# Rita-zi/WavTokenizer

Hardware: AMD Instinct MI355X
Metric: audio-seconds/sec encode+decode, 24 kHz 3 s clips (higher is better)
Workload: dtype f32 (split-f16 x3 products)

## Files before the change

### wavtokenizer_amd/csrc/lstm_persist.hip

```cpp
#include "common.h"

#include <stdlib.h>

namespace wt {

typedef float f32x4p __attribute__((ext_vector_type(4)));
typedef _Float16 f16x8p __attribute__((ext_vector_type(8)));

static constexpr int PW = 12;
static constexpr int HROW = 2 * 2048;
static constexpr int HPITCH = HROW;
template <bool SMALL> __device__ __forceinline__ int lp_swz(int row) { return (SMALL ? 2 * row : row) & 15; }
static constexpr long SPIN_LIMIT_DF = 1L << 20;
template <bool SMALL> struct LpCfg { static constexpr int NLDS = SMALL ? 8 : 6, HROWS = SMALL ? 8 : 16, POLL = SMALL ? 3 : 1; };

__device__ __forceinline__ float sigm_p(float x) { return __builtin_amdgcn_rcpf(1.f + __expf(-x)); }
__device__ __forceinline__ float tanh_p(float x) {
    const float ax = fabsf(x);
    const float e = __expf(-2.f * ax);
    const float t = ax < 0.04f ? ax * (1.f - ax * ax * (1.f / 3.f)) : (1.f - e) * __builtin_amdgcn_rcpf(1.f + e);
    return copysignf(t, x);
}

__device__ __forceinline__ unsigned has_mark(unsigned d) { return (~d - 0x00010001u) & d & 0x80008000u; }
__device__ __forceinline__ _Float16 no_mark(_Float16 v) {
    const unsigned short b = __builtin_bit_cast(unsigned short, v);
    return __builtin_bit_cast(_Float16, (unsigned short)(b == 0xFFFFu ? 0x7E00u : b));
}

#define LP_TRACE(ph) do { if (TRACE && tr_on && s >= 64 && s < 72) { \
    const unsigned long long tt = __builtin_amdgcn_s_memrealtime(); \
    if (lane == 0) { a.ctl[520 + ((s - 64) * 6 + (ph)) * 2] = (unsigned)tt; a.ctl[521 + ((s - 64) * 6 + (ph)) * 2] = (unsigned)(tt >> 32); } } } while (0)
template <bool SMALL, bool TRACE = false>
__global__ __launch_bounds__(64 * PW) void lstm_persist_kernel(const LstmPersistArgs a) {
    constexpr int NBUF = 3;
    constexpr int NLDS = LpCfg<SMALL>::NLDS, HROWS = LpCfg<SMALL>::HROWS;
    extern __shared__ __attribute__((aligned(16))) char sm_p[];
    char* hst = sm_p;
    float* gbuf = reinterpret_cast<float*>(sm_p + HROWS * HPITCH);
    f32x4p* wlds = reinterpret_cast<f32x4p*>(sm_p + HROWS * HPITCH + 3 * 4 * 16 * 17 * sizeof(float)) + (threadIdx.x >> 6) * NLDS * 64 + (threadIdx.x & 63);
    __shared__ unsigned s_xcc, s_w, s_stop;
    const int tid = threadIdx.x, lane = tid & 63, wave = tid >> 6;
    const int role = wave >> 2, ntile = wave & 3;
    const int li = lane & 15, lk = lane >> 4;
    if (tid == 0) {
        const unsigned xcc = __builtin_amdgcn_s_getreg(20 | (3 << 11)) & 7;
        s_xcc = xcc;
        s_w = __hip_atomic_fetch_add(a.ctl + xcc * 32, 1u, __ATOMIC_RELAXED, __HIP_MEMORY_SCOPE_WORKGROUP) + 1u;
        s_stop = 0;
    }
    __syncthreads();
    const int xcc = (int)s_xcc, w = (int)s_w;
    if (w >= 32) return;
    const int H = 512, B = a.B, L = a.L;
    const int c0g = xcc * a.Bx;
    const int nb = B - c0g < a.Bx ? B - c0g : a.Bx;
    if (nb <= 0) return;
    unsigned* err = a.ctl + 512;
    char* hx = reinterpret_cast<char*>(a.hx) + (size_t)xcc * (NBUF * 2 * 16 * 2048);
    const __amdgpu_buffer_rsrc_t rsH = __builtin_amdgcn_make_buffer_rsrc(hx, 0, NBUF * 2 * 16 * 2048, 0x00020000);

    f16x8p wh[16], wl[16 - NLDS];
    {
        const f32x4p* wp = reinterpret_cast<const f32x4p*>(a.Wp) + ((((size_t)role * 32 + w) * 4 + ntile) * 16 * 2) * 64 + lane;
#pragma unroll
        for (int blk = 0; blk < 16; ++blk) {
            wh[blk] = __builtin_bit_cast(f16x8p, wp[(blk * 2 + 0) * 64]);
            if (blk < 16 - NLDS) wl[blk] = __builtin_bit_cast(f16x8p, wp[(blk * 2 + 1) * 64]);
            else wlds[(blk - (16 - NLDS)) * 64] = wp[(blk * 2 + 1) * 64];
        }
    }
    const int c_layer = tid >> 8, c_clip = (tid >> 4) & 15, c_unit = tid & 15;
    const bool c_thr = tid < 512 && c_clip < nb;
    const int c_nt = c_unit >> 2, c_u4 = c_unit & 3;
    const int j = 16 * w + c_unit;
    const long gclip = c0g + c_clip;
    float cst = 0.f;

    for (int e = tid; e < HROWS * HPITCH / 16; e += 64 * PW) reinterpret_cast<f32x4p*>(hst)[e] = (f32x4p){0.f, 0.f, 0.f, 0.f};
    __syncthreads();
    const long spin_limit_df = SPIN_LIMIT_DF >> a.dbg_spin_shift;
    const bool tr_on = TRACE && xcc == 0 && w == 0 && __builtin_amdgcn_readfirstlane(wave) == 0;
    for (int s = 0; s <= L; ++s) {
        LP_TRACE(0);
        float xg[4] = {0.f, 0.f, 0.f, 0.f};
        float xs = 0.f;
        if (c_thr && c_layer == 0 && s < L) {
#pragma unroll
            for (int g = 0; g < 4; ++g) xg[g] = a.xg0[((long)s * B + gclip) * (4 * H) + 64 * w + 16 * c_nt + g * 4 + c_u4];
        }
        if (c_thr && c_layer == 1 && s >= 1) {
            xs = a.x[(gclip * L + (s - 1)) * H + j];
#pragma unroll
            for (int g = 0; g < 4; ++g) xg[g] = a.b1[64 * w + 16 * c_nt + g * 4 + c_u4];
        }

        {
            const int rb = (s + 2) % 3, tot = 2 * nb * 128;
            constexpr int POLL = LpCfg<SMALL>::POLL;
            for (int e0 = tid; e0 < tot; e0 += POLL * 64 * PW) {
                f32x4p v[POLL];
                unsigned need = 0;
#pragma unroll
                for (int it = 0; it < POLL; ++it) {
                    const int e = e0 + it * 64 * PW;
                    if (e < tot && s >= 1 + (e >> 7) / nb) need |= 1u << it;
                }
                unsigned pend = need;
                long spin = 0;
                while (pend) {
#pragma unroll
                    for (int it = 0; it < POLL; ++it)
                        if (pend >> it & 1) {
                            const int e = e0 + it * 64 * PW;
                            const int c16 = e & 127, lc = e >> 7, layer = lc / nb, clip = lc - layer * nb;
                            v[it] = __builtin_bit_cast(f32x4p, __builtin_amdgcn_raw_buffer_load_b128(
                                        rsH, ((rb * 2 + layer) * 16 + clip) * 2048 + c16 * 16, 0, 16 ));
                        }
                    unsigned still = 0;
#pragma unroll
                    for (int it = 0; it < POLL; ++it)
                        if (pend >> it & 1) {
                            const unsigned m = has_mark(__builtin_bit_cast(unsigned, v[it].x)) | has_mark(__builtin_bit_cast(unsigned, v[it].y)) |
                                               has_mark(__builtin_bit_cast(unsigned, v[it].z)) | has_mark(__builtin_bit_cast(unsigned, v[it].w));
                            if (m) still |= 1u << it;
                        }
                    pend = still;
                    if (pend) {
                        if (++spin > spin_limit_df || ((spin & 1023) == 0 && __hip_atomic_load(err, __ATOMIC_RELAXED, __HIP_MEMORY_SCOPE_AGENT) == 1u)) {
                            __hip_atomic_store(err, 1u, __ATOMIC_RELAXED, __HIP_MEMORY_SCOPE_AGENT);
                            if (a.status) __hip_atomic_fetch_or(a.status, (unsigned)WT_STATUS_LSTM, __ATOMIC_RELAXED, __HIP_MEMORY_SCOPE_AGENT);
                            s_stop = 1;
                            break;
                        }
                        __builtin_amdgcn_s_sleep(1);
                    }
                }
#pragma unroll
                for (int it = 0; it < POLL; ++it) {
                    const int e = e0 + it * 64 * PW;
                    if (e < tot) {
                        const int c16 = e & 127, lc = e >> 7, layer = lc / nb, clip = lc - layer * nb;
                        *reinterpret_cast<f32x4p*>(hst + clip * HPITCH + layer * 2048 + ((c16 ^ lp_swz<SMALL>(clip)) * 16)) =
                            (need >> it & 1) ? v[it] : (f32x4p){0.f, 0.f, 0.f, 0.f};
                    }
                }
            }
            LP_TRACE(1);
            __syncthreads();
            LP_TRACE(2);
            if (s_stop) return;
            if (c_thr) {
                unsigned short* mrow = reinterpret_cast<unsigned short*>(hx + ((((s + 1) % 3) * 2 + c_layer) * 16 + c_clip) * 2048);
                mrow[(j >> 5) * 64 + (j & 31)] = 0xFFFFu;
                mrow[(j >> 5) * 64 + 32 + (j & 31)] = 0xFFFFu;
            }
        }
        {
            const bool act = role == 0 ? (s < L) : (s >= 1);
            if (act && SMALL) {
                const int ach = (lk + ((li & 8) ? 4 : 0)) ^ lp_swz<SMALL>(li & 7);
                const char* ap0 = hst + (li & 7) * HPITCH + (role == 2 ? 2048 : 0) + (ach & 7) * 16;
                const char* ape = ap0 + (ach >> 3) * 128;
                const char* apo = ap0 + (1 ^ (ach >> 3)) * 128;
                const bool arow = (li & 7) < nb;
                f32x4p accm = {0.f, 0.f, 0.f, 0.f}, accc = accm;
                f16x8p a1b[2] = {{0, 0, 0, 0, 0, 0, 0, 0}, {0, 0, 0, 0, 0, 0, 0, 0}};
                if (arow) a1b[0] = *reinterpret_cast<const f16x8p*>(ape);
#pragma unroll
                for (int blk = 0; blk < 16; ++blk) {
                    if (blk + 1 < 16 && arow) a1b[(blk + 1) & 1] = *reinterpret_cast<const f16x8p*>((((blk + 1) & 1) ? apo : ape) + ((blk + 1) >> 1) * 256);
                    const f16x8p a1 = a1b[blk & 1];
                    const f16x8p wlb = blk < 16 - NLDS ? wl[blk < 16 - NLDS ? blk : 0]
                                                       : __builtin_bit_cast(f16x8p, wlds[(blk - (16 - NLDS)) * 64]);
                    accm = __builtin_amdgcn_mfma_f32_16x16x32_f16(a1, wh[blk], accm, 0, 0, 0);
                    accc = __builtin_amdgcn_mfma_f32_16x16x32_f16(a1, wlb, accc, 0, 0, 0);
                }
                float* gb = gbuf + ((role * 4 + ntile) * 16) * 17;
#pragma unroll
                for (int r = 0; r < 4; ++r) {
                    const float c2 = __shfl_down(accm[r], 32, 64);
                    if (lk < 2) gb[(4 * lk + r) * 17 + li] = accm[r] + (accc[r] + c2) * (1.f / 2048.f);
                }
            } else if (act) {
                const int ch_h = lk ^ lp_swz<SMALL>(li);
                const char* ap0 = hst + li * HPITCH + (role == 2 ? 2048 : 0) + (ch_h & 7) * 16;
                const char* ape = ap0 + (ch_h >> 3) * 128;
                const char* apo = ap0 + (1 ^ (ch_h >> 3)) * 128;
                const int lo_d = (ch_h & 4) ? -64 : 64;
                f32x4p accm = {0.f, 0.f, 0.f, 0.f}, acc_hl = accm, acc_lh = accm;
                {
                    f16x8p ahb[2];
                    ahb[0] = *reinterpret_cast<const f16x8p*>(ape);
#pragma unroll
                    for (int blk = 0; blk < 16; ++blk) {
                        if (blk + 1 < 16) ahb[(blk + 1) & 1] = *reinterpret_cast<const f16x8p*>((((blk + 1) & 1) ? apo : ape) + ((blk + 1) >> 1) * 256);
                        const f16x8p ah = ahb[blk & 1];
                        const f16x8p wlb = blk < 16 - NLDS ? wl[blk < 16 - NLDS ? blk : 0]
                                                           : __builtin_bit_cast(f16x8p, wlds[(blk - (16 - NLDS)) * 64]);
                        accm = __builtin_amdgcn_mfma_f32_16x16x32_f16(ah, wh[blk], accm, 0, 0, 0);
                        acc_hl = __builtin_amdgcn_mfma_f32_16x16x32_f16(ah, wlb, acc_hl, 0, 0, 0);
                    }
                }
                {
                    f16x8p alb[2];
                    alb[0] = *reinterpret_cast<const f16x8p*>(ape + lo_d);
#pragma unroll
                    for (int blk = 0; blk < 16; ++blk) {
                        if (blk + 1 < 16) alb[(blk + 1) & 1] = *reinterpret_cast<const f16x8p*>((((blk + 1) & 1) ? apo : ape) + ((blk + 1) >> 1) * 256 + lo_d);
                        acc_lh = __builtin_amdgcn_mfma_f32_16x16x32_f16(alb[blk & 1], wh[blk], acc_lh, 0, 0, 0);
                    }
                }
                float* gb = gbuf + ((role * 4 + ntile) * 16) * 17;
#pragma unroll
                for (int r = 0; r < 4; ++r) gb[(4 * lk + r) * 17 + li] = accm[r] + (acc_hl[r] + acc_lh[r]) * (1.f / 2048.f);
            }
        }
        LP_TRACE(3);
        __syncthreads();
        LP_TRACE(4);
        if (c_thr && (c_layer == 0 ? (s < L) : (s >= 1))) {
            float pre[4];
#pragma unroll
            for (int g = 0; g < 4; ++g) {
                const int col = g * 4 + c_u4;
                if (c_layer == 0) pre[g] = gbuf[((0 * 4 + c_nt) * 16 + c_clip) * 17 + col] + xg[g];
                else pre[g] = (gbuf[((1 * 4 + c_nt) * 16 + c_clip) * 17 + col] + gbuf[((2 * 4 + c_nt) * 16 + c_clip) * 17 + col]) + xg[g];
            }
            const float ig = sigm_p(pre[0]), fg = sigm_p(pre[1]), gg = tanh_p(pre[2]), og = sigm_p(pre[3]);
            cst = fg * cst + ig * gg;
            const float h = og * tanh_p(cst);
            _Float16* hrow = reinterpret_cast<_Float16*>(hx + (((s % 3) * 2 + c_layer) * 16 + c_clip) * 2048);
            const _Float16 hh = (_Float16)h;
            const _Float16 hl = (_Float16)((h - (float)hh) * 2048.f);
            __builtin_amdgcn_s_waitcnt(0);
            hrow[(j >> 5) * 64 + (j & 31)] = no_mark(hh);
            hrow[(j >> 5) * 64 + 32 + (j & 31)] = no_mark(hl);
            if (c_layer == 1) {
                const int t = s - 1;
                const float yv = h + xs;
                const float o = a.elu_out ? (yv > 0.f ? yv : __expf(yv) - 1.f) : yv;
                float* yrow = a.y + (gclip * L + t) * H;
                if (a.out_s32) {
                    if (fabsf(o) >= 65504.f && a.status)
                        __hip_atomic_fetch_or(a.status, (unsigned)WT_STATUS_RANGE, __ATOMIC_RELAXED, __HIP_MEMORY_SCOPE_AGENT);
                    _Float16* yp = reinterpret_cast<_Float16*>(yrow) + ((j >> 5) * 64 + (j & 31));
                    const _Float16 oh = (_Float16)o;
                    yp[0] = oh;
                    yp[32] = (_Float16)((o - (float)oh) * 2048.f);
                } else {
                    yrow[j] = o;
                }
            }
        }
        LP_TRACE(5);
    }
}

size_t lstm_persist_hx_bytes() { return (size_t)8 * 3 * 2 * 16 * 2048; }
size_t lstm_persist_ctl_bytes() { return 1024 * sizeof(unsigned); }

int launch_lstm_persist(const LstmPersistArgs& a, hipStream_t stream) {
    if (a.H != 512) { set_error("lstm_persist: built for hidden size 512"); return -1; }
    if (a.B < 1 || a.Bx < 1 || a.Bx > 16 || 8 * a.Bx < a.B) { set_error("lstm_persist: at most 16 clips per XCD (B <= 128)"); return -1; }
    static PerDeviceOnce attr_once;
    constexpr size_t smem_big = (size_t)16 * HPITCH + (size_t)3 * 4 * 16 * 17 * sizeof(float) + (size_t)PW * LpCfg<false>::NLDS * 1024;
    constexpr size_t smem_small = (size_t)8 * HPITCH + (size_t)3 * 4 * 16 * 17 * sizeof(float) + (size_t)PW * LpCfg<true>::NLDS * 1024;
    static_assert(smem_big + 64 <= 160 * 1024 && smem_small + 64 <= 160 * 1024, "LDS budget");
    if (int rc = attr_once.run([&]() -> int {
        WT_HIP_CHECK(hipFuncSetAttribute(reinterpret_cast<const void*>(lstm_persist_kernel<false>), hipFuncAttributeMaxDynamicSharedMemorySize, (int)smem_big));
        WT_HIP_CHECK(hipFuncSetAttribute(reinterpret_cast<const void*>(lstm_persist_kernel<true>), hipFuncAttributeMaxDynamicSharedMemorySize, (int)smem_small));
#ifdef WT_LAB
        WT_HIP_CHECK(hipFuncSetAttribute(reinterpret_cast<const void*>(lstm_persist_kernel<false, true>), hipFuncAttributeMaxDynamicSharedMemorySize, (int)smem_big));
        WT_HIP_CHECK(hipFuncSetAttribute(reinterpret_cast<const void*>(lstm_persist_kernel<true, true>), hipFuncAttributeMaxDynamicSharedMemorySize, (int)smem_small));
#endif
        return 0;
    })) return rc;
    const bool small = a.Bx <= 8;
    LstmPersistArgs b = a;
    if (!b.status) b.status = g_launch.status;
    const char* fault = lab_env("WT_LSTM_PERSIST_FAULT");
    const bool forced = fault && fault[0] == '1';
    if (forced) b.dbg_spin_shift = 8;
    const dim3 grid(forced ? 248 : 256), block(64 * PW);
#ifdef WT_LAB
    if (a.data_flag & 4) {
        if (small) hipLaunchKernelGGL((lstm_persist_kernel<true, true>), grid, block, smem_small, stream, b);
        else hipLaunchKernelGGL((lstm_persist_kernel<false, true>), grid, block, smem_big, stream, b);
    } else
#endif
    {
        if (small) hipLaunchKernelGGL((lstm_persist_kernel<true>), grid, block, smem_small, stream, b);
        else hipLaunchKernelGGL((lstm_persist_kernel<false>), grid, block, smem_big, stream, b);
    }
    WT_HIP_CHECK(hipGetLastError());
    if (LstmForm* f = g_launch.lstm_form) {
        f->kernel = 0; f->small = small ? 1 : 0; f->Bx = a.Bx; f->grid[0] = grid.x; f->grid[1] = grid.y; f->block = block.x;
        f->lds = (unsigned)(small ? smem_small : smem_big);
        ++f->launches;
    }
    return 0;
}

}
```

Baseline: 38340.

## Software-pipeline LDS reads with explicit waitcnt in persistent LSTM step

Rewrites the per-step MFMA loop of the persistent LSTM kernel to issue LDS operand reads through inline ds_read_b128 with fixed offsets. Each read is placed three blocks ahead and guarded by a computed lgkmcnt wait, and the large and small paths are unified into one 32- or 16-block sequence. The polling loop now always issues all POLL loads, decodes the layer with a compare instead of a division and uses a wider POLL for the big config. Cell indices and output offsets are precomputed before the barriers to cut register pressure, and the small config keeps one fewer weight fragment in LDS. Hand-written waitcnt counts are fragile and could break if the compiler reorders LDS operations, and lab-only ablation variants are added.

```diff
diff --git a/wavtokenizer_amd/csrc/lstm_persist.hip b/wavtokenizer_amd/csrc/lstm_persist.hip
--- a/wavtokenizer_amd/csrc/lstm_persist.hip
+++ b/wavtokenizer_amd/csrc/lstm_persist.hip
@@ -1,6 +1,8 @@
 #include "common.h"
 
 #include <stdlib.h>
+
+#include <utility>
 
 namespace wt {
 
@@ -12,7 +14,34 @@
 static constexpr int HPITCH = HROW;
 template <bool SMALL> __device__ __forceinline__ int lp_swz(int row) { return (SMALL ? 2 * row : row) & 15; }
 static constexpr long SPIN_LIMIT_DF = 1L << 20;
-template <bool SMALL> struct LpCfg { static constexpr int NLDS = SMALL ? 8 : 6, HROWS = SMALL ? 8 : 16, POLL = SMALL ? 3 : 1; };
+template <bool SMALL> struct LpCfg { static constexpr int NLDS = SMALL ? 7 : 6, HROWS = SMALL ? 8 : 16, POLL = 3; };
+
+__device__ __forceinline__ unsigned lds_addr(const void* p) { return (unsigned)(size_t)p; }
+template <int OFF> __device__ __forceinline__ void lds_read16(f16x8p& d, unsigned addr) {
+    static_assert(OFF >= 0 && OFF < 65536, "ds offset field");
+    asm volatile("ds_read_b128 %0, %1 offset:%2" : "=v"(d) : "v"(addr), "n"(OFF));
+}
+template <int N> __device__ __forceinline__ void lds_wait(f16x8p& x) { asm volatile("s_waitcnt lgkmcnt(%1)" : "+v"(x) : "n"(N)); }
+template <int N> __device__ __forceinline__ void lds_wait(f16x8p& x, f16x8p& y) { asm volatile("s_waitcnt lgkmcnt(%2)" : "+v"(x), "+v"(y) : "n"(N)); }
+constexpr int lp_ord_a(int k) { return k < 3 ? k : 3 + 2 * (k - 3); }
+constexpr int lp_ord_w(int k) { return 3 + 2 * (k - 2) + 1; }
+constexpr int lp_younger(int v, int NV, int W0) {
+    int last = lp_ord_a(v);
+    if (v >= W0 && v < 16 && lp_ord_w(v) > last) last = lp_ord_w(v);
+    int n = 0;
+    for (int k = 0; k < NV; ++k) if ((k < 3 || k - 3 < v) && lp_ord_a(k) > last) ++n;
+    for (int k = W0; k < 16; ++k) if (k - 2 < v && lp_ord_w(k) > last) ++n;
+    return n;
+}
+__device__ __forceinline__ int lp_fresh(int t) { asm volatile("" : "+v"(t)); return t; }
+#define LP_CELL_IDS \
+    const int c_t = lp_fresh(tid), c_layer = c_t >> 8, c_clip = (c_t >> 4) & 15, c_unit = c_t & 15; \
+    const bool c_thr = c_t < 512 && c_clip < nb; \
+    const int c_nt = c_unit >> 2, c_u4 = c_unit & 3; \
+    const int j = 16 * w + c_unit;                        \
+    const long gclip = c0g + c_clip; \
+    (void)c_layer; (void)c_nt; (void)c_u4; (void)j; (void)gclip
+template <class F, int... I> __device__ __forceinline__ void lp_blocks(F&& f, std::integer_sequence<int, I...>) { (f(std::integral_constant<int, I>{}), ...); }
 
 __device__ __forceinline__ float sigm_p(float x) { return __builtin_amdgcn_rcpf(1.f + __expf(-x)); }
 __device__ __forceinline__ float tanh_p(float x) {
@@ -30,19 +59,17 @@
 
 #define LP_TRACE(ph) do { if (TRACE && tr_on && s >= 64 && s < 72) { \
     const unsigned long long tt = __builtin_amdgcn_s_memrealtime(); \
-    if (lane == 0) { a.ctl[520 + ((s - 64) * 6 + (ph)) * 2] = (unsigned)tt; a.ctl[521 + ((s - 64) * 6 + (ph)) * 2] = (unsigned)(tt >> 32); } } } while (0)
-template <bool SMALL, bool TRACE = false>
+    if ((tid & 63) == 0) { a.ctl[520 + ((s - 64) * 6 + (ph)) * 2] = (unsigned)tt; a.ctl[521 + ((s - 64) * 6 + (ph)) * 2] = (unsigned)(tt >> 32); } } } while (0)
+template <bool SMALL, bool TRACE = false, int ABL = 0>
 __global__ __launch_bounds__(64 * PW) void lstm_persist_kernel(const LstmPersistArgs a) {
     constexpr int NBUF = 3;
     constexpr int NLDS = LpCfg<SMALL>::NLDS, HROWS = LpCfg<SMALL>::HROWS;
     extern __shared__ __attribute__((aligned(16))) char sm_p[];
     char* hst = sm_p;
     float* gbuf = reinterpret_cast<float*>(sm_p + HROWS * HPITCH);
-    f32x4p* wlds = reinterpret_cast<f32x4p*>(sm_p + HROWS * HPITCH + 3 * 4 * 16 * 17 * sizeof(float)) + (threadIdx.x >> 6) * NLDS * 64 + (threadIdx.x & 63);
+    char* wlds0 = sm_p + HROWS * HPITCH + 3 * 4 * 16 * 17 * sizeof(float);
     __shared__ unsigned s_xcc, s_w, s_stop;
     const int tid = threadIdx.x, lane = tid & 63, wave = tid >> 6;
-    const int role = wave >> 2, ntile = wave & 3;
-    const int li = lane & 15, lk = lane >> 4;
     if (tid == 0) {
         const unsigned xcc = __builtin_amdgcn_s_getreg(20 | (3 << 11)) & 7;
         s_xcc = xcc;
@@ -62,7 +89,9 @@
 
     f16x8p wh[16], wl[16 - NLDS];
     {
+        const int role = wave >> 2, ntile = wave & 3;
         const f32x4p* wp = reinterpret_cast<const f32x4p*>(a.Wp) + ((((size_t)role * 32 + w) * 4 + ntile) * 16 * 2) * 64 + lane;
+        f32x4p* wlds = reinterpret_cast<f32x4p*>(wlds0) + wave * NLDS * 64 + lane;
 #pragma unroll
         for (int blk = 0; blk < 16; ++blk) {
             wh[blk] = __builtin_bit_cast(f16x8p, wp[(blk * 2 + 0) * 64]);
@@ -70,186 +99,204 @@
             else wlds[(blk - (16 - NLDS)) * 64] = wp[(blk * 2 + 1) * 64];
         }
     }
-    const int c_layer = tid >> 8, c_clip = (tid >> 4) & 15, c_unit = tid & 15;
-    const bool c_thr = tid < 512 && c_clip < nb;
-    const int c_nt = c_unit >> 2, c_u4 = c_unit & 3;
-    const int j = 16 * w + c_unit;
-    const long gclip = c0g + c_clip;
     float cst = 0.f;
 
     for (int e = tid; e < HROWS * HPITCH / 16; e += 64 * PW) reinterpret_cast<f32x4p*>(hst)[e] = (f32x4p){0.f, 0.f, 0.f, 0.f};
     __syncthreads();
-    const long spin_limit_df = SPIN_LIMIT_DF >> a.dbg_spin_shift;
+    const int spin_limit_df = (int)(SPIN_LIMIT_DF >> a.dbg_spin_shift);
     const bool tr_on = TRACE && xcc == 0 && w == 0 && __builtin_amdgcn_readfirstlane(wave) == 0;
     for (int s = 0; s <= L; ++s) {
         LP_TRACE(0);
         float xg[4] = {0.f, 0.f, 0.f, 0.f};
         float xs = 0.f;
-        if (c_thr && c_layer == 0 && s < L) {
-#pragma unroll
-            for (int g = 0; g < 4; ++g) xg[g] = a.xg0[((long)s * B + gclip) * (4 * H) + 64 * w + 16 * c_nt + g * 4 + c_u4];
-        }
-        if (c_thr && c_layer == 1 && s >= 1) {
-            xs = a.x[(gclip * L + (s - 1)) * H + j];
-#pragma unroll
-            for (int g = 0; g < 4; ++g) xg[g] = a.b1[64 * w + 16 * c_nt + g * 4 + c_u4];
-        }
-
+        unsigned ape, apo, apw;
+        int lo_d;
         {
             const int rb = (s + 2) % 3, tot = 2 * nb * 128;
             constexpr int POLL = LpCfg<SMALL>::POLL;
-            for (int e0 = tid; e0 < tot; e0 += POLL * 64 * PW) {
-                f32x4p v[POLL];
+            for (int e0 = lp_fresh(tid); e0 < tot; e0 += POLL * 64 * PW) {
                 unsigned need = 0;
+                int off[POLL];
 #pragma unroll
                 for (int it = 0; it < POLL; ++it) {
-                    const int e = e0 + it * 64 * PW;
-                    if (e < tot && s >= 1 + (e >> 7) / nb) need |= 1u << it;
-                }
-                unsigned pend = need;
-                long spin = 0;
-                while (pend) {
+                    const int e = e0 + it * 64 * PW, ec = e < tot ? e : tot - 1;
+                    const int c16 = ec & 127, lc = ec >> 7, layer = lc >= nb ? 1 : 0, clip = lc - layer * nb;
+                    off[it] = ((rb * 2 + layer) * 16 + clip) * 2048 + c16 * 16;
+                    if (e < tot && s >= 1 + layer) need |= 1u << it;
+                }
+                f32x4p va[POLL];
+                int spin = 0;
+                while (need) {
 #pragma unroll
                     for (int it = 0; it < POLL; ++it)
-                        if (pend >> it & 1) {
-                            const int e = e0 + it * 64 * PW;
-                            const int c16 = e & 127, lc = e >> 7, layer = lc / nb, clip = lc - layer * nb;
-                            v[it] = __builtin_bit_cast(f32x4p, __builtin_amdgcn_raw_buffer_load_b128(
-                                        rsH, ((rb * 2 + layer) * 16 + clip) * 2048 + c16 * 16, 0, 16 ));
-                        }
+                        va[it] = __builtin_bit_cast(f32x4p, __builtin_amdgcn_raw_buffer_load_b128(rsH, off[it], 0, 16 ));
                     unsigned still = 0;
 #pragma unroll
-                    for (int it = 0; it < POLL; ++it)
-                        if (pend >> it & 1) {
-                            const unsigned m = has_mark(__builtin_bit_cast(unsigned, v[it].x)) | has_mark(__builtin_bit_cast(unsigned, v[it].y)) |
-                                               has_mark(__builtin_bit_cast(unsigned, v[it].z)) | has_mark(__builtin_bit_cast(unsigned, v[it].w));
-                            if (m) still |= 1u << it;
-                        }
-                    pend = still;
-                    if (pend) {
-                        if (++spin > spin_limit_df || ((spin & 1023) == 0 && __hip_atomic_load(err, __ATOMIC_RELAXED, __HIP_MEMORY_SCOPE_AGENT) == 1u)) {
-                            __hip_atomic_store(err, 1u, __ATOMIC_RELAXED, __HIP_MEMORY_SCOPE_AGENT);
-                            if (a.status) __hip_atomic_fetch_or(a.status, (unsigned)WT_STATUS_LSTM, __ATOMIC_RELAXED, __HIP_MEMORY_SCOPE_AGENT);
-                            s_stop = 1;
-                            break;
-                        }
-                        __builtin_amdgcn_s_sleep(1);
-                    }
+                    for (int it = 0; it < POLL; ++it) {
+                        const unsigned m = has_mark(__builtin_bit_cast(unsigned, va[it].x)) | has_mark(__builtin_bit_cast(unsigned, va[it].y)) |
+                                           has_mark(__builtin_bit_cast(unsigned, va[it].z)) | has_mark(__builtin_bit_cast(unsigned, va[it].w));
+                        if (m) still |= 1u << it;
+                    }
+                    if ((ABL & 2) || !(still & need)) break;
+                    if (++spin > spin_limit_df || ((spin & 1023) == 0 && __hip_atomic_load(err, __ATOMIC_RELAXED, __HIP_MEMORY_SCOPE_AGENT) == 1u)) {
+                        __hip_atomic_store(err, 1u, __ATOMIC_RELAXED, __HIP_MEMORY_SCOPE_AGENT);
+                        if (a.status) __hip_atomic_fetch_or(a.status, (unsigned)WT_STATUS_LSTM, __ATOMIC_RELAXED, __HIP_MEMORY_SCOPE_AGENT);
+                        s_stop = 1;
+                        break;
+                    }
+                    __builtin_amdgcn_s_sleep(1);
                 }
 #pragma unroll
                 for (int it = 0; it < POLL; ++it) {
                     const int e = e0 + it * 64 * PW;
                     if (e < tot) {
-                        const int c16 = e & 127, lc = e >> 7, layer = lc / nb, clip = lc - layer * nb;
+                        const int c16 = e & 127, lc = e >> 7, layer = lc >= nb ? 1 : 0, clip = lc - layer * nb;
                         *reinterpret_cast<f32x4p*>(hst + clip * HPITCH + layer * 2048 + ((c16 ^ lp_swz<SMALL>(clip)) * 16)) =
-                            (need >> it & 1) ? v[it] : (f32x4p){0.f, 0.f, 0.f, 0.f};
-                    }
-                }
-            }
+                            (need >> it & 1) ? va[it] : (f32x4p){0.f, 0.f, 0.f, 0.f};
+                    }
+                }
+            }
+            {
+                LP_CELL_IDS;
+                if (c_thr && c_layer == 0 && s < L) {
+#pragma unroll
+                    for (int g = 0; g < 4; ++g) xg[g] = a.xg0[((long)s * B + gclip) * (4 * H) + 64 * w + 16 * c_nt + g * 4 + c_u4];
+                }
+                if (c_thr && c_layer == 1 && s >= 1) {
+                    xs = a.x[(gclip * L + (s - 1)) * H + j];
+#pragma unroll
+                    for (int g = 0; g < 4; ++g) xg[g] = a.b1[64 * w + 16 * c_nt + g * 4 + c_u4];
+                }
+            }
+            int m_off;
+            {
+                LP_CELL_IDS;
+                m_off = c_thr ? ((((s + 1) % 3) * 2 + c_layer) * 16 + c_clip) * 2048 + ((j >> 5) * 64 + (j & 31)) * 2 : -1;
+            }
+            {
+                const int tp = lp_fresh(tid), role = tp >> 8, li = tp & 15, lk = (tp >> 4) & 3;
+                const int row = SMALL ? (li & 7) : li;
+                const int ch = (SMALL ? lk + ((li & 8) ? 4 : 0) : lk) ^ lp_swz<SMALL>(row);
+                const unsigned ap0 = lds_addr(hst + row * HPITCH + (role == 2 ? 2048 : 0) + (ch & 7) * 16);
+                ape = ap0 + (ch >> 3) * 128;
+                apo = ap0 + (1 ^ (ch >> 3)) * 128;
+                lo_d = (ch & 4) ? -64 : 64;
+                apw = lds_addr(wlds0) + (tp >> 6) * (NLDS * 1024) + (tp & 63) * 16;
+            }
+            asm volatile("" : "+v"(m_off), "+v"(ape), "+v"(apo), "+v"(lo_d), "+v"(apw));
             LP_TRACE(1);
             __syncthreads();
             LP_TRACE(2);
             if (s_stop) return;
-            if (c_thr) {
-                unsigned short* mrow = reinterpret_cast<unsigned short*>(hx + ((((s + 1) % 3) * 2 + c_layer) * 16 + c_clip) * 2048);
-                mrow[(j >> 5) * 64 + (j & 31)] = 0xFFFFu;
-                mrow[(j >> 5) * 64 + 32 + (j & 31)] = 0xFFFFu;
+            if (m_off >= 0) {
+                unsigned short* mrow = reinterpret_cast<unsigned short*>(hx + m_off);
+                mrow[0] = 0xFFFFu;
+                mrow[32] = 0xFFFFu;
             }
         }
         {
+            const int tp = lp_fresh(tid), role = tp >> 8, ntile = (tp >> 6) & 3, li = tp & 15, lk = (tp >> 4) & 3;
             const bool act = role == 0 ? (s < L) : (s >= 1);
-            if (act && SMALL) {
-                const int ach = (lk + ((li & 8) ? 4 : 0)) ^ lp_swz<SMALL>(li & 7);
-                const char* ap0 = hst + (li & 7) * HPITCH + (role == 2 ? 2048 : 0) + (ach & 7) * 16;
-                const char* ape = ap0 + (ach >> 3) * 128;
-                const char* apo = ap0 + (1 ^ (ach >> 3)) * 128;
-                const bool arow = (li & 7) < nb;
-                f32x4p accm = {0.f, 0.f, 0.f, 0.f}, accc = accm;
-                f16x8p a1b[2] = {{0, 0, 0, 0, 0, 0, 0, 0}, {0, 0, 0, 0, 0, 0, 0, 0}};
-                if (arow) a1b[0] = *reinterpret_cast<const f16x8p*>(ape);
-#pragma unroll
-                for (int blk = 0; blk < 16; ++blk) {
-                    if (blk + 1 < 16 && arow) a1b[(blk + 1) & 1] = *reinterpret_cast<const f16x8p*>((((blk + 1) & 1) ? apo : ape) + ((blk + 1) >> 1) * 256);
-                    const f16x8p a1 = a1b[blk & 1];
-                    const f16x8p wlb = blk < 16 - NLDS ? wl[blk < 16 - NLDS ? blk : 0]
-                                                       : __builtin_bit_cast(f16x8p, wlds[(blk - (16 - NLDS)) * 64]);
-                    accm = __builtin_amdgcn_mfma_f32_16x16x32_f16(a1, wh[blk], accm, 0, 0, 0);
-                    accc = __builtin_amdgcn_mfma_f32_16x16x32_f16(a1, wlb, accc, 0, 0, 0);
-                }
+            if (act) {
+                constexpr int NV = SMALL ? 16 : 32, W0 = 16 - NLDS;
+                static_assert(W0 >= 2 && NLDS >= 1, "the first lo-weight fragment is requested behind block W0 - 2");
+                f32x4p accm = {0.f, 0.f, 0.f, 0.f}, acc2 = accm, acc_lh = accm;
+                f16x8p ar[3], wr[2];
+                auto read_a = [&](auto vc) {
+                    constexpr int v = decltype(vc)::value, blk = v & 15;
+                    lds_read16<(blk >> 1) * 256>(ar[v % 3], ((blk & 1) ? apo : ape) + (v >= 16 ? lo_d : 0));
+                };
+                auto read_w = [&](auto kc) {
+                    constexpr int k = decltype(kc)::value;
+                    lds_read16<(k - W0) * 1024>(wr[k & 1], apw);
+                };
+                asm volatile("s_waitcnt lgkmcnt(0)" ::: "memory");
+                if (ABL & 1) {
+                    lp_blocks(read_a, std::make_integer_sequence<int, NV>{});
+                    lp_blocks([&](auto kc) { read_w(std::integral_constant<int, W0 + decltype(kc)::value>{}); }, std::make_integer_sequence<int, NLDS>{});
+                    lds_wait<0>(ar[0], ar[1]);
+                    lds_wait<0>(ar[2], wr[0]);
+                    lds_wait<0>(wr[1]);
+                } else {
+                    read_a(std::integral_constant<int, 0>{});
+                    read_a(std::integral_constant<int, 1>{});
+                    read_a(std::integral_constant<int, 2>{});
+                }
+                lp_blocks([&](auto vc) {
+                    constexpr int v = decltype(vc)::value;
+                    constexpr bool lds_w = v >= W0 && v < 16;
+                    if constexpr (!(ABL & 1)) {
+                        if constexpr (lds_w) lds_wait<lp_younger(v, NV, W0)>(ar[v % 3], wr[v & 1]);
+                        else lds_wait<lp_younger(v, NV, W0)>(ar[v % 3]);
+                    }
+                    const f16x8p av = ar[v % 3];
+                    if constexpr (v < 16) {
+                        const f16x8p wlb = lds_w ? wr[v & 1] : wl[v < W0 ? v : 0];
+                        accm = __builtin_amdgcn_mfma_f32_16x16x32_f16(av, wh[v], accm, 0, 0, 0);
+                        acc2 = __builtin_amdgcn_mfma_f32_16x16x32_f16(av, wlb, acc2, 0, 0, 0);
+                    } else {
+                        acc_lh = __builtin_amdgcn_mfma_f32_16x16x32_f16(av, wh[v & 15], acc_lh, 0, 0, 0);
+                    }
+                    if constexpr (!(ABL & 1)) {
+                        if constexpr (v + 3 < NV) read_a(std::integral_constant<int, v + 3>{});
+                        if constexpr (v + 2 >= W0 && v + 2 < 16) read_w(std::integral_constant<int, v + 2>{});
+                    }
+                }, std::make_integer_sequence<int, NV>{});
                 float* gb = gbuf + ((role * 4 + ntile) * 16) * 17;
-#pragma unroll
-                for (int r = 0; r < 4; ++r) {
-                    const float c2 = __shfl_down(accm[r], 32, 64);
-                    if (lk < 2) gb[(4 * lk + r) * 17 + li] = accm[r] + (accc[r] + c2) * (1.f / 2048.f);
-                }
-            } else if (act) {
-                const int ch_h = lk ^ lp_swz<SMALL>(li);
-                const char* ap0 = hst + li * HPITCH + (role == 2 ? 2048 : 0) + (ch_h & 7) * 16;
-                const char* ape = ap0 + (ch_h >> 3) * 128;
-                const char* apo = ap0 + (1 ^ (ch_h >> 3)) * 128;
-                const int lo_d = (ch_h & 4) ? -64 : 64;
-                f32x4p accm = {0.f, 0.f, 0.f, 0.f}, acc_hl = accm, acc_lh = accm;
-                {
-                    f16x8p ahb[2];
-                    ahb[0] = *reinterpret_cast<const f16x8p*>(ape);
-#pragma unroll
-                    for (int blk = 0; blk < 16; ++blk) {
-                        if (blk + 1 < 16) ahb[(blk + 1) & 1] = *reinterpret_cast<const f16x8p*>((((blk + 1) & 1) ? apo : ape) + ((blk + 1) >> 1) * 256);
-                        const f16x8p ah = ahb[blk & 1];
-                        const f16x8p wlb = blk < 16 - NLDS ? wl[blk < 16 - NLDS ? blk : 0]
-                                                           : __builtin_bit_cast(f16x8p, wlds[(blk - (16 - NLDS)) * 64]);
-                        accm = __builtin_amdgcn_mfma_f32_16x16x32_f16(ah, wh[blk], accm, 0, 0, 0);
-                        acc_hl = __builtin_amdgcn_mfma_f32_16x16x32_f16(ah, wlb, acc_hl, 0, 0, 0);
-                    }
-                }
-                {
-                    f16x8p alb[2];
-                    alb[0] = *reinterpret_cast<const f16x8p*>(ape + lo_d);
-#pragma unroll
-                    for (int blk = 0; blk < 16; ++blk) {
-                        if (blk + 1 < 16) alb[(blk + 1) & 1] = *reinterpret_cast<const f16x8p*>((((blk + 1) & 1) ? apo : ape) + ((blk + 1) >> 1) * 256 + lo_d);
-                        acc_lh = __builtin_amdgcn_mfma_f32_16x16x32_f16(alb[blk & 1], wh[blk], acc_lh, 0, 0, 0);
-                    }
-                }
-                float* gb = gbuf + ((role * 4 + ntile) * 16) * 17;
-#pragma unroll
-                for (int r = 0; r < 4; ++r) gb[(4 * lk + r) * 17 + li] = accm[r] + (acc_hl[r] + acc_lh[r]) * (1.f / 2048.f);
-            }
-        }
+                if (SMALL) {
+#pragma unroll
+                    for (int r = 0; r < 4; ++r) {
+                        const float c2 = __shfl_down(accm[r], 32, 64);
+                        if (lk < 2) gb[(4 * lk + r) * 17 + li] = accm[r] + (acc2[r] + c2) * (1.f / 2048.f);
+                    }
+                } else {
+#pragma unroll
+                    for (int r = 0; r < 4; ++r) gb[(4 * lk + r) * 17 + li] = accm[r] + (acc2[r] + acc_lh[r]) * (1.f / 2048.f);
+                }
+            }
+        }
+        int c_gi, c_hoff, c_kind;
+        long c_yoff;
+        {
+            LP_CELL_IDS;
+            c_kind = !(c_thr && (c_layer == 0 ? (s < L) : (s >= 1))) ? 0 : 1 + c_layer;
+            c_gi = ((c_layer * 4 + c_nt) * 16 + c_clip) * 17 + c_u4;
+            c_hoff = (((s % 3) * 2 + c_layer) * 16 + c_clip) * 2048 + ((j >> 5) * 64 + (j & 31)) * 2;
+            c_yoff = (gclip * L + (s - 1)) * H * 4 + (a.out_s32 ? ((j >> 5) * 64 + (j & 31)) * 2 : j * 4);
+        }
+        asm volatile("" : "+v"(c_gi), "+v"(c_hoff), "+v"(c_kind), "+v"(c_yoff));
         LP_TRACE(3);
         __syncthreads();
         LP_TRACE(4);
-        if (c_thr && (c_layer == 0 ? (s < L) : (s >= 1))) {
+        if (c_kind) {
             float pre[4];
 #pragma unroll
             for (int g = 0; g < 4; ++g) {
-                const int col = g * 4 + c_u4;
-                if (c_layer == 0) pre[g] = gbuf[((0 * 4 + c_nt) * 16 + c_clip) * 17 + col] + xg[g];
-                else pre[g] = (gbuf[((1 * 4 + c_nt) * 16 + c_clip) * 17 + col] + gbuf[((2 * 4 + c_nt) * 16 + c_clip) * 17 + col]) + xg[g];
+                if (c_kind == 1) pre[g] = gbuf[c_gi + g * 4] + xg[g];
+                else pre[g] = (gbuf[c_gi + g * 4] + gbuf[c_gi + 4 * 16 * 17 + g * 4]) + xg[g];
             }
             const float ig = sigm_p(pre[0]), fg = sigm_p(pre[1]), gg = tanh_p(pre[2]), og = sigm_p(pre[3]);
             cst = fg * cst + ig * gg;
             const float h = og * tanh_p(cst);
-            _Float16* hrow = reinterpret_cast<_Float16*>(hx + (((s % 3) * 2 + c_layer) * 16 + c_clip) * 2048);
+            _Float16* hrow = reinterpret_cast<_Float16*>(hx + c_hoff);
             const _Float16 hh = (_Float16)h;
             const _Float16 hl = (_Float16)((h - (float)hh) * 2048.f);
             __builtin_amdgcn_s_waitcnt(0);
-            hrow[(j >> 5) * 64 + (j & 31)] = no_mark(hh);
-            hrow[(j >> 5) * 64 + 32 + (j & 31)] = no_mark(hl);
-            if (c_layer == 1) {
-                const int t = s - 1;
+            hrow[0] = no_mark(hh);
+            hrow[32] = no_mark(hl);
+            if (c_kind == 2) {
                 const float yv = h + xs;
                 const float o = a.elu_out ? (yv > 0.f ? yv : __expf(yv) - 1.f) : yv;
-                float* yrow = a.y + (gclip * L + t) * H;
+                char* yb = reinterpret_cast<char*>(a.y) + c_yoff;
                 if (a.out_s32) {
                     if (fabsf(o) >= 65504.f && a.status)
                         __hip_atomic_fetch_or(a.status, (unsigned)WT_STATUS_RANGE, __ATOMIC_RELAXED, __HIP_MEMORY_SCOPE_AGENT);
-                    _Float16* yp = reinterpret_cast<_Float16*>(yrow) + ((j >> 5) * 64 + (j & 31));
+                    _Float16* yp = reinterpret_cast<_Float16*>(yb);
                     const _Float16 oh = (_Float16)o;
                     yp[0] = oh;
                     yp[32] = (_Float16)((o - (float)oh) * 2048.f);
                 } else {
-                    yrow[j] = o;
+                    *reinterpret_cast<float*>(yb) = o;
                 }
             }
         }
@@ -273,6 +320,10 @@
 #ifdef WT_LAB
         WT_HIP_CHECK(hipFuncSetAttribute(reinterpret_cast<const void*>(lstm_persist_kernel<false, true>), hipFuncAttributeMaxDynamicSharedMemorySize, (int)smem_big));
         WT_HIP_CHECK(hipFuncSetAttribute(reinterpret_cast<const void*>(lstm_persist_kernel<true, true>), hipFuncAttributeMaxDynamicSharedMemorySize, (int)smem_small));
+        WT_HIP_CHECK(hipFuncSetAttribute(reinterpret_cast<const void*>(lstm_persist_kernel<false, true, 1>), hipFuncAttributeMaxDynamicSharedMemorySize, (int)smem_big));
+        WT_HIP_CHECK(hipFuncSetAttribute(reinterpret_cast<const void*>(lstm_persist_kernel<true, true, 1>), hipFuncAttributeMaxDynamicSharedMemorySize, (int)smem_small));
+        WT_HIP_CHECK(hipFuncSetAttribute(reinterpret_cast<const void*>(lstm_persist_kernel<false, true, 2>), hipFuncAttributeMaxDynamicSharedMemorySize, (int)smem_big));
+        WT_HIP_CHECK(hipFuncSetAttribute(reinterpret_cast<const void*>(lstm_persist_kernel<true, true, 2>), hipFuncAttributeMaxDynamicSharedMemorySize, (int)smem_small));
 #endif
         return 0;
     })) return rc;
@@ -285,8 +336,14 @@
     const dim3 grid(forced ? 248 : 256), block(64 * PW);
 #ifdef WT_LAB
     if (a.data_flag & 4) {
-        if (small) hipLaunchKernelGGL((lstm_persist_kernel<true, true>), grid, block, smem_small, stream, b);
-        else hipLaunchKernelGGL((lstm_persist_kernel<false, true>), grid, block, smem_big, stream, b);
+        const char* e = lab_env("WT_LSTM_ABL");
+        const int abl = e ? atoi(e) : 0;
+        if (abl != 0 && abl != 1 && abl != 2) { set_error("lstm_persist: WT_LSTM_ABL is 0, 1 or 2"); return -1; }
+        void (*kern)(const LstmPersistArgs) =
+            abl == 1 ? (small ? lstm_persist_kernel<true, true, 1> : lstm_persist_kernel<false, true, 1>)
+          : abl == 2 ? (small ? lstm_persist_kernel<true, true, 2> : lstm_persist_kernel<false, true, 2>)
+                     : (small ? lstm_persist_kernel<true, true> : lstm_persist_kernel<false, true>);
+        hipLaunchKernelGGL(kern, grid, block, small ? smem_small : smem_big, stream, b);
     } else
 #endif
     {
```

Result: no change. 38100 (-0.6%).
